# Prayforhanluo/HiCHap_master

Measured on AMD Instinct MI355X. Metric: ICE iterations/sec on 10 kb whole-genome matrix (also nnz*iters/sec), higher is better.
Workload: dtype f64; 1 GPU; hg19-10kb-diploid-wholegenome; n_bins=607282, nnz_upper=4998527599, resolution_bp=10000, parallelism=single GPU, entries_stored=9997055198, slots_u32=160483740, slots_u16=3332512024, payload_bytes=14837255808, tiles=88993, units=88985, hbm_bytes_matrix=15785038153

## Files before the change

### hichap_master_amd/csrc/ice.hip

```cpp
#include <algorithm>
#include <chrono>
#include <functional>
#include <cmath>
#include <limits>

#include "ice_internal.hpp"

namespace hh {
constexpr int kThreads = 256;

constexpr int kSweepThreads = 512;
constexpr int kSweepWaves = kSweepThreads / 64;
constexpr int kFlatU = 8;
static_assert(kFlatU == kFlatIlvU, "k_sweep_flatw walks the interleaved layout's runs");

__device__ __forceinline__ double lds_b(const double* bl, uint32_t byteoff) {
    return *reinterpret_cast<const double*>(reinterpret_cast<const char*>(bl) + byteoff);
}

__device__ __forceinline__ void tile_dot(const uint4 v, const double* __restrict__ bl, double& a0, double& a1) {
    const uint32_t w[4] = {v.x, v.y, v.z, v.w};
    double x[4];
#pragma unroll
    for (int i = 0; i < 4; ++i) x[i] = lds_b(bl, w[i] & 0xFFFFu);
// ... 1179 lines not shown
                {
                    double w[G / 2];
#pragma unroll
                    for (int k = 0; k < G / 2; ++k) w[k] = b0[G / 2 + k];
#pragma unroll
                    for (int j = 0; j < RJ; ++j) acc[j] = band_dot_half<BITS, 1>(sh[j], w, acc[j]);
                }
            }
        }
#pragma unroll
        for (int j = 0; j < RJ; ++j) {
            const double t = wave_sum(acc[j]);
            if (lane == 0 && a[j]) out[r0 + gb + wave + NW * (j0 + j)] = t;
        }
    }
}

template <int ROWS>
struct BandLds {
    static constexpr int L8 = BandGeo<8, ROWS>::LDS, L4 = BandGeo<4, ROWS>::LDS;
    double bl[L8 > L4 ? L8 : L4];
    uint8_t ract[ROWS];
};

template <int ABL, int ROWS, bool DPP = true>
__device__ __forceinline__ void band_any(const BandSegs& S, int rblk, int y, BandLds<ROWS>& L, long long nloc,
                                         long long row_lo, long long n_bins, const uint8_t* __restrict__ act,
                                         const uint16_t* __restrict__ row_group, const double* __restrict__ b,
                                         double* __restrict__ bpart) {
    const int c = S.ord[y];
    int k = 0;
    while (k + 1 < S.n && c >= S.s[k + 1].ch) ++k;
    const BandSeg P = S.s[k];
    if (P.bits == 8)
        band_block<8, ABL, ROWS, DPP>(P, rblk, c - P.ch, L.bl, L.ract, nloc, row_lo, n_bins, act, row_group, b, bpart);
    else
        band_block<4, ABL, ROWS, DPP>(P, rblk, c - P.ch, L.bl, L.ract, nloc, row_lo, n_bins, act, row_group, b, bpart);
}

template <int ABL, int ROWS, bool DPP = true>
__global__ __launch_bounds__(kBandThreads, 4) void k_sweep_bands(BandSegs S, long long nloc, long long row_lo,
                                                              long long n_bins, const uint8_t* __restrict__ act,
                                                              const uint16_t* __restrict__ row_group,
                                                              const double* __restrict__ b,
                                                              double* __restrict__ bpart) {
    __shared__ BandLds<ROWS> L;
    band_any<ABL, ROWS, DPP>(S, blockIdx.x, blockIdx.y, L, nloc, row_lo, n_bins, act, row_group, b, bpart);
}

constexpr int kUbRows = 128;
constexpr int kUbWaves = 4;
constexpr int kUbThreads = 64 * kUbWaves;
constexpr int kUbGroupRows = kUbRows * kUbWaves;
constexpr int kUbChunk = 1008;
constexpr int kUbCols = kUbGroupRows + kUbChunk;
static_assert(kR % kUbGroupRows == 0, "upper-band workgroups must not straddle a shard's row-block boundary");
constexpr int kUbTails = (kUbChunk + kUbGroupRows - 1) / kUbGroupRows;
constexpr int kUbArrs = 2 + kUbTails;
constexpr int kMaxUbChunks = 40;

struct UbSeg {
    const uint8_t* loc;
    const uint8_t* halo;
    long long stride;
    long long dlo;
    int bytes;
    int nc, ch, bits;
};
struct UbSegs {
    UbSeg s[2];
    int n;
    uint8_t ord[kMaxUbChunks];
};
struct UbArgs {
    long long row_lo, row_hi, halo_lo, nloc, g_lo;
    const uint8_t* act;
    const uint16_t* row_group;
    const double* b;
    double* upart;
};

template <int BITS>
struct UbT;
template <>
struct UbT<8> {
    typedef uint4 V;
    static constexpr int LB = 16;
    static __device__ __forceinline__ V zero() { return make_uint4(0u, 0u, 0u, 0u); }
    static __device__ __forceinline__ V ld(const uint8_t* p) { return ld16(reinterpret_cast<const uint4*>(p)); }
    template <int M>
    static __device__ __forceinline__ V shift(const V prev, const V own) {
        if (M == 0) return own;
        constexpr int B = 128 - 8 * M;
        return band_shift_q<B / 32>(prev, own, B % 32);
    }
    static __device__ __forceinline__ uint32_t cnt(const V v, int k) {
        const uint32_t x = k < 4 ? v.x : k < 8 ? v.y : k < 12 ? v.z : v.w;
        return (x >> (8 * (k & 3))) & 0xFFu;
    }
};
typedef uint32_t u32x2 __attribute__((ext_vector_type(2)));
template <>
struct UbT<4> {
    typedef uint2 V;
    static constexpr int LB = 8;
    static __device__ __forceinline__ V zero() { return make_uint2(0u, 0u); }
    static __device__ __forceinline__ V ld(const uint8_t* p) {
        const u32x2 v = *reinterpret_cast<const u32x2*>(p);
        return make_uint2(v.x, v.y);
    }
    template <int M>
    static __device__ __forceinline__ V shift(const V prev, const V own) {
        if (M == 0) return own;
        constexpr int B = 64 - 4 * M, Q = B / 32, R = B % 32;
        const uint32_t d[4] = {prev.x, prev.y, own.x, own.y};
        if (R == 0) return make_uint2(d[Q], d[Q + 1]);
        return make_uint2(__builtin_amdgcn_alignbit(d[Q + 1], d[Q], R), __builtin_amdgcn_alignbit(d[Q + 2], d[Q + 1], R));
    }
    static __device__ __forceinline__ uint32_t cnt(const V v, int k) {
        return ((k < 8 ? v.x : v.y) >> (4 * (k & 7))) & 0xFu;
    }
};

__device__ __forceinline__ double dpp_shl1_d(double x) {
    const int lo = __builtin_amdgcn_update_dpp(0, __double2loint(x), 0x130, 0xF, 0xF, false);
    const int hi = __builtin_amdgcn_update_dpp(0, __double2hiint(x), 0x130, 0xF, 0xF, false);
    return __hiloint2double(hi, lo);
}

__device__ __forceinline__ double ub_cvt(uint32_t x) {
    double r;
    asm volatile("v_cvt_f64_u32 %0, %1" : "=v"(r) : "v"(x));
    return r;
}

__device__ __forceinline__ double ub_bias(const double* __restrict__ b, long long c, long long n) {
    const bool in = c >= 0 && c < n;
    const double v = b[in ? c : 0];
    return (in && v == v) ? v : 0.0;
}

template <int H, int MASK>
__device__ __forceinline__ void ub_halve(double (&v)[8], int lane) {
    const bool hi = (lane & MASK) != 0;
#pragma unroll
    for (int j = 0; j < H; ++j) {
        const double send = hi ? v[j] : v[j + H];
        const double keep = hi ? v[j + H] : v[j];
        v[j] = keep + __shfl_xor(send, MASK, 64);
    }
}
__device__ __forceinline__ double ub_reduce8(double (&v)[8], int lane) {
    ub_halve<4, 1>(v, lane);
    ub_halve<2, 2>(v, lane);
    ub_halve<1, 4>(v, lane);
    double x = v[0];
    x += __shfl_xor(x, 8, 64);
    x += __shfl_xor(x, 16, 64);
    x += __shfl_xor(x, 32, 64);
    return x;
}
__device__ __forceinline__ int ub_reduce8_row(int lane) { return (lane & 1) * 4 + (lane & 2) + ((lane >> 2) & 1); }

__device__ __forceinline__ int ub_pad(int j) { return j + (j >> 4); }
constexpr int kUbWin = kUbCols + kUbCols / 16 + 1;

template <int BITS>
__device__ __forceinline__ void ub_walk(const UbSeg& P, int kc, int chunk, long long r0, const UbArgs& a,
                                        long long n_bins, double* __restrict__ heads, double (&col)[16],
                                        const double* __restrict__ cwin, const double* __restrict__ rowb) {
    using T = UbT<BITS>;
    using V = typename T::V;
    const int lane = threadIdx.x & 63;
    int cb = (kc * kUbChunk + 16 * (lane - 1)) * BITS / 8;
    const bool outside = cb < 0 || cb >= P.bytes;
    const uint32_t msk = (BITS == 8 && outside) ? 0u : ~0u;
    if (outside) cb = P.bytes - T::LB;
    const long long rhi = a.row_hi < r0 + kUbRows ? a.row_hi : r0 + kUbRows;
    const int nv = (int)(rhi - r0);
    const uint8_t* __restrict__ rows = (r0 >= a.row_lo ? P.loc + (r0 - a.row_lo) * P.stride
                                                       : P.halo + (r0 - a.halo_lo) * P.stride) + cb;
    const long long stride = P.stride;
    auto load_row = [&](int i) -> V { return T::ld(rows + (long long)(i < nv ? i : nv - 1) * stride); };
    const int wo = (int)(r0 % kUbGroupRows);
    double w[16];
#pragma unroll
    for (int k = 0; k < 16; ++k) col[k] = 0.0;
    double* __restrict__ R = a.upart + (size_t)(kUbArrs * chunk) * a.nloc;
    V buf[2][4];
#pragma unroll
    for (int j = 0; j < 4; ++j) buf[0][j] = load_row(j);
// ... 5 lines not shown
            {
                const double* src = cwin + ub_pad(wo + 16 * g + 16 * (lane > 0 ? lane - 1 : 0));
#pragma unroll
                for (int k = 0; k < 16; ++k) w[k] = lane ? src[k] : 0.0;
            }
#pragma unroll
            for (int h = 0; h < 2; ++h) {
                double racc[8];
#pragma unroll
                for (int q = 0; q < 2; ++q) {
                    const int bt = 2 * h + q;
#pragma unroll
                    for (int j = 0; j < 4; ++j) buf[(bt + 1) & 1][j] = load_row(16 * g + 4 * (bt + 1) + j);
#pragma unroll
                    for (int j = 0; j < 4; ++j) {
                        const int m = 4 * bt + j, mm = 4 * q + j;
                        V own = buf[bt & 1][j];
                        if (BITS == 8) {
                            uint4& o = *reinterpret_cast<uint4*>(&own);
                            o.x &= msk;
                            o.y &= msk;
                            o.z &= msk;
                            o.w &= msk;
                        }
                        V prev;
                        if (BITS == 8) {
                            const uint4 o = *reinterpret_cast<const uint4*>(&own);
                            const uint4 pv = dpp_shr1(o);
                            prev = *reinterpret_cast<const V*>(&pv);
                        } else {
                            const uint2 o = *reinterpret_cast<const uint2*>(&own);
                            const uint2 pv = make_uint2(__builtin_amdgcn_update_dpp(0u, o.x, 0x138, 0xF, 0xF, false),
                                                        __builtin_amdgcn_update_dpp(0u, o.y, 0x138, 0xF, 0xF, false));
                            prev = *reinterpret_cast<const V*>(&pv);
                        }
                        V sh;
                        switch (m) {
                            case 0: sh = T::template shift<0>(prev, own); break;
                            case 1: sh = T::template shift<1>(prev, own); break;
                            case 2: sh = T::template shift<2>(prev, own); break;
                            case 3: sh = T::template shift<3>(prev, own); break;
                            case 4: sh = T::template shift<4>(prev, own); break;
                            case 5: sh = T::template shift<5>(prev, own); break;
                            case 6: sh = T::template shift<6>(prev, own); break;
                            case 7: sh = T::template shift<7>(prev, own); break;
                            case 8: sh = T::template shift<8>(prev, own); break;
                            case 9: sh = T::template shift<9>(prev, own); break;
                            case 10: sh = T::template shift<10>(prev, own); break;
                            case 11: sh = T::template shift<11>(prev, own); break;
                            case 12: sh = T::template shift<12>(prev, own); break;
                            case 13: sh = T::template shift<13>(prev, own); break;
                            case 14: sh = T::template shift<14>(prev, own); break;
                            default: sh = T::template shift<15>(prev, own); break;
                        }
                        const double br = rowb[wo + 16 * g + m];
                        double a0 = 0.0, a1 = 0.0;
#pragma unroll
                        for (int k = 0; k < 16; k += 2) {
                            const double c0 = ub_cvt(T::cnt(sh, k)), c1 = ub_cvt(T::cnt(sh, k + 1));
                            a0 = fma(c0, w[k], a0);
                            a1 = fma(c1, w[k + 1], a1);
                            col[k] = fma(c0, br, col[k]);
                            col[k + 1] = fma(c1, br, col[k + 1]);
                            asm volatile("" : "+v"(col[k]), "+v"(col[k + 1]), "+v"(a0), "+v"(a1));
                        }
                        racc[mm] = a0 + a1;
                    }
                    __builtin_amdgcn_sched_barrier(0);
                }
                const double s = ub_reduce8(racc, lane);
                const long long r = gb + 8 * h + ub_reduce8_row(lane);
                if (lane < 8 && r < rhi && r >= a.row_lo) R[r - a.row_lo] = s;
            }
        }
        if (lane == 1) {
#pragma unroll
            for (int k = 0; k < 16; ++k) heads[16 * g + k] = col[k];
        }
#pragma unroll
        for (int k = 0; k < 16; ++k) col[k] = dpp_shl1_d(col[k]);
    }
}

__device__ __forceinline__ void ub_group(const UbSegs& S, long long grp, int chunk, const UbArgs& a, long long n_bins,
                                         double* __restrict__ cbuf, double* __restrict__ cwin,
                                         double* __restrict__ rowb) {
    int si = 0;
    while (si + 1 < S.n && chunk >= S.s[si + 1].ch) ++si;
    const UbSeg& P = S.s[si];
    const int kc = chunk - P.ch;
    const long long R0 = grp * kUbGroupRows;
    const int wave = __builtin_amdgcn_readfirstlane(threadIdx.x >> 6), lane = threadIdx.x & 63;
    const long long base = P.dlo + (long long)kc * kUbChunk;
    for (int j = threadIdx.x; j < kUbCols - kUbGroupRows; j += kUbThreads) cbuf[kUbGroupRows + j] = 0.0;
    for (int j = threadIdx.x; j < kUbCols; j += kUbThreads) cwin[ub_pad(j)] = ub_bias(a.b, R0 + base + j, n_bins);
    for (int j = threadIdx.x; j < kUbGroupRows; j += kUbThreads) rowb[j] = ub_bias(a.b, R0 + j, n_bins);
    __syncthreads();
    const long long r0 = R0 + (long long)kUbRows * wave;
    const bool rows_here = r0 < a.row_hi && r0 + kUbRows > a.row_lo;
    const bool cols_here = r0 + base < a.row_hi && r0 + kUbRows + base + kUbChunk > a.row_lo;
    const bool stored = r0 + kUbRows > a.halo_lo && r0 < a.row_hi;
    double col[16];
    double* heads = cbuf + (size_t)kUbRows * wave;
    if ((rows_here || cols_here) && stored) {
        if (P.bits == 8)
            ub_walk<8>(P, kc, chunk, r0, a, n_bins, heads, col, cwin, rowb);
        else
            ub_walk<4>(P, kc, chunk, r0, a, n_bins, heads, col, cwin, rowb);
    } else {
        for (int j = lane; j < kUbRows; j += 64) heads[j] = 0.0;
#pragma unroll
        for (int k = 0; k < 16; ++k) col[k] = 0.0;
    }
    for (int w = 0; w < kUbWaves; ++w) {
        __syncthreads();
        if (wave == w && lane > 0) {
            double* t = cbuf + (size_t)kUbRows * (wave + 1) + 16 * (lane - 1);
#pragma unroll
            for (int k = 0; k < 16; ++k) t[k] += col[k];
        }
    }
    __syncthreads();
    double* __restrict__ base_p = a.upart + (size_t)(kUbArrs * chunk + 1) * a.nloc;
    for (int j = threadIdx.x; j < kUbCols; j += kUbThreads) {
        const long long c = R0 + base + j;
        if (c >= a.row_lo && c < a.row_hi) base_p[(size_t)(j / kUbGroupRows) * a.nloc + (c - a.row_lo)] = cbuf[j];
    }
}

__global__ __launch_bounds__(kUbThreads, 3) void k_sweep_ubands(UbSegs S, UbArgs a, long long n_bins, int xcd) {
    __shared__ double cbuf[kUbCols];
    __shared__ double cwin[kUbWin];
    __shared__ double rowb[kUbGroupRows];
    long long grp = blockIdx.x;
    int y = blockIdx.y;
    if (xcd) {
        const long long nb = (long long)gridDim.x * gridDim.y, b = blockIdx.x + (long long)blockIdx.y * gridDim.x;
        const long long L = xcd_remap(b, nb);
        y = (int)(L % gridDim.y);
        grp = L / gridDim.y;
    }
    ub_group(S, a.g_lo + grp, S.ord[y], a, n_bins, cbuf, cwin, rowb);
}

__global__ void k_ub_halo(const uint8_t* __restrict__ band, const uint8_t* __restrict__ band4, long long W8,
                          long long W4, long long row_lo, long long row_hi, long long halo_lo,
                          uint8_t* __restrict__ h8, uint8_t* __restrict__ h4) {
    const long long nh = row_lo - halo_lo;
    const long long st8 = band_stride(W8), st4 = band4_stride(W8, W4), sg = band4_seg(W8, W4);
    const long long per = W8 + (W4 > W8 ? sg : 0);
    const long long i = (long long)blockIdx.x * blockDim.x + threadIdx.x;
    if (i >= nh * per) return;
    const long long hr = i / per, j = i % per, c = halo_lo + hr;
    if (j < W8) {
        const long long d = j + 1, r = c + d;
        if (r >= row_lo && r < row_hi) h8[hr * st8 + W8 + d] = band[(r - row_lo) * st8 + (W8 - d)];
    } else {
        const long long jb = j - W8;
        uint32_t v = 0;
#pragma unroll
        for (int q = 0; q < 2; ++q) {
            const long long d = W8 + 1 + 2 * jb + q, r = c + d;
            if (d <= W4 && r >= row_lo && r < row_hi) {
                const long long nib = band4_nibble(-d, W8, W4);
                v |= ((band4[(r - row_lo) * st4 + (nib >> 1)] >> (4 * (nib & 1))) & 0xFu) << (4 * q);
            }
        }
        h4[hr * st4 + sg + jb] = (uint8_t)v;
    }
}

static_assert(kBandThreads == kSweepThreads, "one block shape");
template <int NB, int U, int ABL, bool UP>
__global__ __launch_bounds__(kSweepThreads, 4) void k_sweep_all(TileDev T, const uint8_t* __restrict__ act,
                                                              int n_tiled, int n_band, BandSegs S, int band_rb,
                                                              long long nloc, long long row_lo,
                                                              const uint16_t* __restrict__ row_group,
                                                              const double* __restrict__ b, long long n_bins,
                                                              double* __restrict__ part,
                                                              double* __restrict__ bpart,
                                                              unsigned long long* __restrict__ trace) {
    __shared__ __attribute__((aligned(16))) union Lds {
        TiledLds<UP> t;
        FlatLds<UP> f;
        BandLds<64> band;
    } L;
    const int x = blockIdx.x;
    const unsigned long long t0 = trace ? wall_clock64() : 0ull;
    if (x < n_tiled) {
        sweep_tiled_unit<NB, ABL, UP>(T, act, T.u_order[x], b, n_bins, part, L.t);
    } else if (x < n_tiled + n_band) {
        const int y = x - n_tiled;
        band_any<ABL, 64>(S, y % band_rb, y / band_rb, L.band, nloc, row_lo, n_bins, act, row_group, b, bpart);
    } else {
        sweep_flat_unit<U, ABL, UP>(T, act, T.u_order[x - n_band], b, n_bins, part, L.f);
    }
    if (trace) {
        __syncthreads();
        if (threadIdx.x == 0) {
            trace[3 * (size_t)x] = t0;
            trace[3 * (size_t)x + 1] = wall_clock64();
            trace[3 * (size_t)x + 2] = (unsigned long long)__smid();
        }
    }
}

struct UbMarg {
    const double* part;
    int n;
    long long base[kMaxUbChunks];
};
constexpr int kMargThreads = kR;
constexpr int kMargU = 256;

struct TileArgs {
    const int32_t* tile_lo;
    const int32_t* tile_hi;
    const int32_t* tile_group;
    const int32_t* group_tile_ptr;
    const int32_t* blk_tile_ptr;
    double* tile_cnt;
    double* tile_sum;
    double* tile_sq;
    double* g_cnt;
    double* g_sum;
// ... 410 lines not shown
constexpr int kFuseMaxTiles = 128;
}

struct hh_ice {
    hh_matrix* m = nullptr;
    hh_ice_opts o{};
    int64_t n = 0, nloc = 0;
    int32_t G = 1;
    std::vector<int64_t> glo, ghi;
    int32_t n_tiles = 0;
    DBuf<int32_t> tile_lo, tile_hi, tile_group, group_tile_ptr, blk_tile_ptr;
    DBuf<double> bias, marg, part, tile_cnt, tile_sum, tile_sq, g_cnt, g_sum;
    DBuf<unsigned> counter;
    bool stats_fresh = false;
    DBuf<double> bpart;
    int32_t nch = 0;
    int32_t nchu = 0;
    DBuf<double> upart;
    DBuf<uint8_t> halo8, halo4;
    int64_t halo_lo = 0, ub_glo = 0, ub_ghi = 0;
    DBuf<uint8_t> active;
    DBuf<double> g_var, g_mean;
    DBuf<int32_t> g_iters;
    DBuf<uint8_t> g_empty;
    DBuf<long long> rank_rows;
    std::vector<int64_t> h_rank_rows;
    DBuf<unsigned long long> colpart, colacc, bmax, bfix;
    DBuf<double> fix;
    double rmax = 1.0;
    bool rmax_global = false;
    int32_t cx_world = 1, cx_rank = 0;
    int64_t cx_maxlen = 0;
    std::vector<int64_t> cx_rr;
    DBuf<long long> cx_rr_dev;
    hh_reduce_fn cx_fn = nullptr;
    void* cx_user = nullptr;
    hh_allgather_fn cx_ag = nullptr;
    void* cx_ag_user = nullptr;
    DBuf<unsigned long long> cx_send, cx_recv, cx_all;
    int32_t iters_done = 0;
    PinnedBuf<uint8_t> h_active;
    std::vector<hipEvent_t> ev;
    double sweep_ms = 0.0, iter_ms = 0.0;
    int32_t sweep_launches = 0;
    hipStream_t side = nullptr, side2 = nullptr;
    hipEvent_t fork = nullptr, join = nullptr, join2 = nullptr;
    ~hh_ice() {
        for (auto e : ev) (void)hipEventDestroy(e);
        if (join2) (void)hipEventDestroy(join2);
        if (side2) (void)hipStreamDestroy(side2);
        if (fork) (void)hipEventDestroy(fork);
        if (join) (void)hipEventDestroy(join);
        if (side) (void)hipStreamDestroy(side);
    }
    bool full() const { return m->row_lo == 0 && m->row_hi == m->n_bins; }
    TileArgs ta() {
        return TileArgs{tile_lo.p, tile_hi.p, tile_group.p, group_tile_ptr.p, blk_tile_ptr.p, tile_cnt.p,
                        tile_sum.p, tile_sq.p, g_cnt.p, g_sum.p, counter.p};
    }
    bool small_stats() const { return hh::g_fuse_stats == 1 || (hh::g_fuse_stats < 0 && n_tiles <= hh::kFuseMaxTiles); }
    uint8_t* act() { return active.p + (iters_done & 1) * G; }
    uint8_t* nxt() { return active.p + (1 - (iters_done & 1)) * G; }
};

namespace hh {

static int g_sweep_nb = 2;
static int g_band_dpp = 0;
static int g_flatw_waves = 11;
static int g_flatw_waves_up = 8;
static int g_flatw_pipe = 2;
static int g_sweep_ablate = 0;
static int g_band_concurrent = 1;
static int g_split_tiles = 1;
static int g_conc_order = 1;
static int64_t g_conc_min_bytes = 8LL << 30;
static int64_t g_conc_ub_min_bytes = 1LL << 30;
static int g_band_rows = 0;
static int g_band_fused = 1;
static int g_band_lpt = 1;
static int g_uband = 1;
static int64_t g_uband_min_bytes = 128LL << 20;
static int g_ub_xcd = 1;
static int g_sweep_single = -1;
static int g_iter_events = 1;
static int64_t g_single_max_bytes = 1LL << 30;
static unsigned long long* g_trace = nullptr;
static int64_t g_trace_cap = 0, g_trace_n = 0;

template <int NB, int ABL, bool UP>
static void launch_sweep_up(const hh_matrix* m, const TileDev& T, const uint8_t* act, const double* b, double* part,
                            hipStream_t s, hipStream_t s_tiled, int which) {
    const int n_tiled = (int)(m->n_units - m->n_units_flat), n_flat = (int)m->n_units_flat;
    auto tiled = [&] {
        if (!n_tiled) return;
        HH_KTIME("k_sweep_tiled", s_tiled);
        hipLaunchKernelGGL((k_sweep_tiled<NB, ABL, UP>), dim3((unsigned)n_tiled), dim3(kSweepThreads), 0, s_tiled,
                           T, act, n_tiled, b, (long long)m->n_bins, part);
    };
    if (which & 1) tiled();
    if (!(which & 2)) return;
    HH_KTIME(n_flat ? "k_sweep_flat" : nullptr, s);
    if (n_flat && m->n_fgroups) {
        HH_REQUIRE(m->flat_perm, "column-grouped flat tiles without the interleaved layout");
        auto kern = g_flatw_pipe == 2   ? k_sweep_flatw<kFlatU, ABL, 2>
                    : g_flatw_pipe == 1 ? k_sweep_flatw<kFlatU, ABL, 1>
                                        : k_sweep_flatw<kFlatU, ABL, 0>;
        int nw = 8;
        if constexpr (UP) {
            nw = g_flatw_waves_up == 11 ? 11 : 8;
            kern = nw == 11 ? k_sweep_flatw<kFlatU, ABL, 2, 11, true> : k_sweep_flatw<kFlatU, ABL, 2, 8, true>;
        } else {
            if (g_flatw_waves == 10) {
                kern = g_flatw_pipe == 2 ? k_sweep_flatw<kFlatU, ABL, 2, 10> : k_sweep_flatw<kFlatU, ABL, 0, 10>;
                nw = 10;
            } else if (g_flatw_waves == 11) {
                kern = g_flatw_pipe == 2 ? k_sweep_flatw<kFlatU, ABL, 2, 11> : k_sweep_flatw<kFlatU, ABL, 0, 11>;
                nw = 11;
            }
        }
        hipLaunchKernelGGL(kern, dim3((unsigned)m->n_fgroups), dim3(64 * nw), 0, s, T, act, b,
                           (long long)m->n_bins, part);
    } else if (n_flat) {
        hipLaunchKernelGGL((k_sweep_flat<kFlatU, ABL, UP>), dim3((unsigned)n_flat), dim3(kSweepThreads), 0, s, T,
                           act, n_flat, n_tiled, b, (long long)m->n_bins, part);
    }
}

template <int NB, int ABL>
static void launch_sweep(const hh_matrix* m, const TileDev& T, const uint8_t* act, const double* b, double* part,
                         hipStream_t s, hipStream_t s_tiled, int which) {
    if constexpr (kUpperBuild) {
        if (T.upper) return launch_sweep_up<NB, ABL, true>(m, T, act, b, part, s, s_tiled, which);
    }
    launch_sweep_up<NB, ABL, false>(m, T, act, b, part, s, s_tiled, which);
}

template <int ABL>
static void launch_sweep_nb(const hh_matrix* m, const TileDev& T, const uint8_t* act, const double* b, double* part,
                            hipStream_t s, hipStream_t st, int which) {
    switch (g_sweep_nb) {
        case 1: launch_sweep<1, ABL>(m, T, act, b, part, s, st, which); break;
        case 2: launch_sweep<2, ABL>(m, T, act, b, part, s, st, which); break;
        case 8: launch_sweep<8, ABL>(m, T, act, b, part, s, st, which); break;
        default: launch_sweep<4, ABL>(m, T, act, b, part, s, st, which); break;
    }
}

static void sweep(const hh_matrix* m, const TileDev& T, const uint8_t* act, const double* b, double* part,
                  hipStream_t s, hipStream_t s_tiled = nullptr, int which = 3) {
    if (m->n_units == 0) return;
    if (!s_tiled) s_tiled = s;
    switch (g_sweep_ablate) {
        case 1: launch_sweep_nb<1>(m, T, act, b, part, s, s_tiled, which); break;
        case 2: launch_sweep_nb<2>(m, T, act, b, part, s, s_tiled, which); break;
        case 3: launch_sweep_nb<3>(m, T, act, b, part, s, s_tiled, which); break;
        default: launch_sweep_nb<0>(m, T, act, b, part, s, s_tiled, which); break;
    }
    HIP_CHECK(hipGetLastError());
}

static TileDev tdev(const hh_ice* S) { return S->m->dev(S->colpart.p, S->fix.p, S->bfix.p); }

static void band_order(BandSegs& segs, int ch) {
    std::vector<std::pair<long long, int>> w;
    for (int k = 0; k < segs.n; ++k)
        for (int c = 0; c < segs.s[k].nc; ++c) {
            const long long bytes = std::min<long long>(kBandChunkB, segs.s[k].bytes - (long long)c * kBandChunkB);
            w.push_back({g_band_lpt ? -bytes * (8 / segs.s[k].bits) : 0, segs.s[k].ch + c});
        }
    std::stable_sort(w.begin(), w.end(), [](const auto& a, const auto& b) { return a.first < b.first; });
    for (int y = 0; y < ch; ++y) segs.ord[y] = (uint8_t)w[y].second;
}

static int band_segs(const hh_matrix* m, BandSegs& segs) {
    const long long W8 = m->band_w, W4 = m->band_w4;
    segs = BandSegs{};
    int ch = 0;
    auto add = [&](const uint8_t* seg, long long stride, long long bytes, long long dlo, int bits) {
        const int nc = (int)((bytes + kBandChunkB - 1) / kBandChunkB);
        segs.s[segs.n++] = BandSeg{seg, stride, dlo, (int)bytes, nc, ch, bits};
        ch += nc;
    };
    if (W8 > 0) add(m->band.p, band_stride(W8), band_stride(W8), -W8, 8);
    if (W4 > W8) {
        const long long st = band4_stride(W8, W4), sg = band4_seg(W8, W4);
        add(m->band4.p, st, sg, -W4, 4);
        add(m->band4.p + sg, st, sg, W8 + 1, 4);
    }
    HH_REQUIRE(ch <= kMaxBandChunks, "too many band chunks");
    band_order(segs, ch);
    return ch;
}

static int ub_segs(const hh_ice* S, UbSegs& u) {
    const hh_matrix* m = S->m;
    const long long W8 = m->band_w, W4 = m->band_w4;
    u = UbSegs{};
    int ch = 0;
    auto add = [&](const uint8_t* loc, const uint8_t* halo, long long stride, long long dlo, long long bytes,
                   long long slots, int bits) {
        const int nc = (int)((slots + 15 + kUbChunk - 1) / kUbChunk);
        u.s[u.n++] = UbSeg{loc, halo, stride, dlo, (int)bytes, nc, ch, bits};
        ch += nc;
    };
    if (W8 > 0)
        add(m->band.p + W8, S->halo8.p ? S->halo8.p + W8 : nullptr, band_stride(W8), 0, W8 + 16, W8 + 1, 8);
    if (W4 > W8) {
        const long long sg = band4_seg(W8, W4);
        add(m->band4.p + sg, S->halo4.p ? S->halo4.p + sg : nullptr, band4_stride(W8, W4), W8 + 1, sg, W4 - W8, 4);
    }
    HH_REQUIRE(ch <= kMaxUbChunks, "too many upper-band chunks");
    std::vector<std::pair<long long, int>> w;
    for (int k = 0; k < u.n; ++k)
        for (int c = 0; c < u.s[k].nc; ++c) {
            const long long slots = u.s[k].bits == 8 ? W8 + 1 : W4 - W8;
            w.push_back({-std::min<long long>(kUbChunk, slots + 15 - (long long)c * kUbChunk), u.s[k].ch + c});
        }
    std::stable_sort(w.begin(), w.end(), [](const auto& a, const auto& b) { return a.first < b.first; });
    for (int y = 0; y < ch; ++y) u.ord[y] = (uint8_t)w[y].second;
    return ch;
}

static UbArgs ub_args(hh_ice* S) {
    const hh_matrix* m = S->m;
    return UbArgs{m->row_lo, m->row_hi, S->halo_lo, S->nloc, S->ub_glo, S->act(), m->row_group.p, S->bias.p,
                  S->upart.p};
}

static UbMarg ub_marg(const hh_ice* S) {
    UbMarg u{};
    u.part = S->upart.p;
    u.n = S->nchu;
    if (!S->nchu) return u;
    UbSegs segs;
    ub_segs(S, segs);
    for (int k = 0; k < segs.n; ++k)
        for (int c = 0; c < segs.s[k].nc; ++c) u.base[segs.s[k].ch + c] = segs.s[k].dlo + (long long)c * kUbChunk;
    return u;
}

static void sweep_uband(hh_ice* S, hipStream_t s) {
    UbSegs segs;
    const int ch = ub_segs(S, segs);
    const long long ng = S->ub_ghi - S->ub_glo;
    if (!ch || ng <= 0) return;
    HH_KTIME("k_sweep_ubands", s);
    hipLaunchKernelGGL(k_sweep_ubands, dim3((unsigned)ng, (unsigned)ch), dim3(kUbThreads), 0, s, segs, ub_args(S),
                       (long long)S->m->n_bins, g_ub_xcd);
    HIP_CHECK(hipGetLastError());
}

static void sweep_band(hh_ice* S, hipStream_t s) {
    if (S->nchu) {
        if (S->nloc) sweep_uband(S, s);
        return;
    }
    const hh_matrix* m = S->m;
    if (!S->nch || !S->nloc) return;
    BandSegs segs;
    const int ch = band_segs(m, segs);
    const int rows = g_band_rows ? g_band_rows : (((S->nloc + 255) / 256) * ch < 1024 ? 64 : 256);
    const bool abl = g_sweep_ablate == 1;
    auto launch = [&](const BandSegs& L, int nc) {
        const unsigned rb = (unsigned)((S->nloc + rows - 1) / rows);
        auto kern = rows == 64    ? (abl ? k_sweep_bands<1, 64> : k_sweep_bands<0, 64>)
                    : rows == 128 ? (abl ? k_sweep_bands<1, 128> : k_sweep_bands<0, 128>)
                                  : (abl ? k_sweep_bands<1, 256>
                                         : (g_band_dpp ? k_sweep_bands<0, 256, true> : k_sweep_bands<0, 256, false>));
        hipLaunchKernelGGL(kern, dim3(rb, (unsigned)nc), dim3(kBandThreads), 0, s, L, (long long)S->nloc,
                           (long long)m->row_lo, (long long)m->n_bins, S->act(), m->row_group.p, S->bias.p,
                           S->bpart.p);
        HIP_CHECK(hipGetLastError());
    };
    if (g_band_fused) {
        launch(segs, ch);
    } else {
        for (int k = 0; k < segs.n; ++k) {
            BandSegs one{};
            one.s[0] = segs.s[k];
            one.n = 1;
            for (int y = 0; y < segs.s[k].nc; ++y) one.ord[y] = (uint8_t)(segs.s[k].ch + y);
            launch(one, segs.s[k].nc);
        }
    }
}

static void sweep_single(hh_ice* S, hipStream_t s) {
    const hh_matrix* m = S->m;
    BandSegs segs;
    const int ch = (S->nch && S->nloc && !S->nchu) ? band_segs(m, segs) : (segs = BandSegs{}, 0);
    const int band_rb = (int)((S->nloc + 63) / 64);
    const int n_tiled = (int)(m->n_units - m->n_units_flat), n_flat = (int)m->n_units_flat;
    const long long n_band = ch ? (long long)band_rb * ch : 0;
    const long long grid = n_tiled + n_band + n_flat;
    if (S->nchu && S->nloc) sweep_uband(S, s);
    if (!grid) return;
    HH_REQUIRE(grid < (1LL << 31), "sweep grid too large for one launch");
    unsigned long long* trace = grid <= g_trace_cap ? g_trace : nullptr;
    if (trace) g_trace_n = grid;
    auto kern = g_sweep_ablate == 1   ? k_sweep_all<2, kFlatU, 1, false>
                : g_sweep_ablate == 2 ? k_sweep_all<2, kFlatU, 2, false>
                                      : k_sweep_all<2, kFlatU, 0, false>;
    if constexpr (kUpperBuild) {
        if (m->upper && S->colpart.p)
            kern = g_sweep_ablate == 1   ? k_sweep_all<2, kFlatU, 1, true>
                   : g_sweep_ablate == 2 ? k_sweep_all<2, kFlatU, 2, true>
                                         : k_sweep_all<2, kFlatU, 0, true>;
    }
    hipLaunchKernelGGL(kern, dim3((unsigned)grid), dim3(kSweepThreads), 0, s, tdev(S), S->act(), n_tiled,
                       (int)n_band, segs, band_rb, (long long)S->nloc, (long long)m->row_lo, m->row_group.p,
                       S->bias.p, (long long)m->n_bins, S->part.p, S->bpart.p, trace);
    HIP_CHECK(hipGetLastError());
}

static void ensure_side_streams(hh_ice* S) {
    if (S->side) return;
    int cur = 0;
    HIP_CHECK(hipGetDevice(&cur));
    if (cur != S->m->device) HIP_CHECK(hipSetDevice(S->m->device));
    HIP_CHECK(hipStreamCreateWithFlags(&S->side, hipStreamNonBlocking));
    HIP_CHECK(hipEventCreateWithFlags(&S->fork, hipEventDisableTiming));
    HIP_CHECK(hipEventCreateWithFlags(&S->join, hipEventDisableTiming));
    HIP_CHECK(hipStreamCreateWithFlags(&S->side2, hipStreamNonBlocking));
    HIP_CHECK(hipEventCreateWithFlags(&S->join2, hipEventDisableTiming));
    if (cur != S->m->device) HIP_CHECK(hipSetDevice(cur));
}

static void marg_weighted(hh_ice* S, double* out, hipStream_t s, bool timed, int slot) {
    hh_matrix* m = S->m;
    const bool up = m->upper && S->colpart.p;
    const bool shard_x = up && S->cx_world > 1;
// ... 144 lines not shown
    const std::vector<double> all = gather ? gather(marg) : marg;
    std::vector<double> logm;
    for (double x : all)
        if (x > 0) logm.push_back(std::log(x));
    const double med = np_median(logm);
    std::vector<double> dev(logm.size());
    for (size_t k = 0; k < logm.size(); ++k) dev[k] = std::fabs(logm[k] - med);
    const double cutoff = std::exp(med - S->o.mad_max * np_median(dev));
    for (int64_t i = 0; i < S->n; ++i)
        if (marg[i] < cutoff) bias[i] = 0.0;
    upload_pinned_sync(S->bias.p, bias.data(), (size_t)S->n, s);
}

extern "C" {

int hh_tune(const char* key, int64_t value) {
    return guard([&] {
        HH_REQUIRE(key, "null key");
        const std::string k(key);
        if (k == "sweep_nb") {
            HH_REQUIRE(value == 1 || value == 2 || value == 4 || value == 8, "sweep_nb must be 1, 2, 4 or 8");
            g_sweep_nb = (int)value;
        } else if (k == "sweep_ablate") {
            HH_REQUIRE(value >= 0 && value <= 3, "sweep_ablate must be 0, 1, 2 or 3");
            g_sweep_ablate = (int)value;
        } else if (k == "band4_density_pct" || k == "band8_big_pct") {
            HH_REQUIRE(value >= 1 && value <= 100, "percent in [1, 100]");
            (k == "band4_density_pct" ? g_band4_density : g_band8_big) = (double)value / 100.0;
        } else if (k == "band4") {
            HH_REQUIRE(value == 0 || value == 1, "band4 in {0, 1}");
            g_band4 = value;
        } else if (k == "flat_cols") {
            HH_REQUIRE(value >= -1 && value <= 1, "flat_cols in {-1 (auto), 0, 1}");
            g_flat_cols = value;
        } else if (k == "flatw_pipe") {
            HH_REQUIRE(value >= 0 && value <= 2, "flatw_pipe in {0, 1, 2}");
            g_flatw_pipe = (int)value;
        } else if (k == "band_dpp") {
            HH_REQUIRE(value == 0 || value == 1, "band_dpp in {0, 1}");
            g_band_dpp = (int)value;
        } else if (k == "flatw_u") {
            HH_REQUIRE(value == 8, "flatw_u: 8 (the interleaved flat layout's run length)");
        } else if (k == "flatw_waves_up") {
            HH_REQUIRE(value == 8 || value == 11, "flatw_waves_up in {8, 11}");
            g_flatw_waves_up = (int)value;
        } else if (k == "upper_tiles") {
            HH_REQUIRE(value >= -1 && value <= 1, "upper_tiles in {-1 (auto), 0, 1}");
            HH_REQUIRE(kUpperBuild || value != 1,
                       "upper-triangle tiles need the 4096-column build (libhichap_hip_up.so, -DHH_KWBITS=12)");
            g_upper_tiles = value;
        } else if (k == "flat_max") {
            HH_REQUIRE(value >= 0 && value <= 255, "flat_max in [0, 255]");
            g_flat_max = value;
        } else if (k == "unit_entries") {
            HH_REQUIRE(value == 0 || (value >= 4096 && value <= (1 << 24)), "unit_entries must be 0 (auto) or in [4096, 2^24]");
            g_unit_entries = value;
        } else if (k == "flat_defer") {
            HH_REQUIRE(value == 0 || value == 1, "flat_defer in {0, 1}");
            g_flat_defer = (int)value;
        } else if (k == "unit_lpt") {
            HH_REQUIRE(value >= 0 && value <= 2, "unit_lpt in {0, 1, 2}");
            g_unit_lpt = value;
        } else if (k == "unit_lpt_lists") {
            HH_REQUIRE(value >= 0 && value <= 3, "unit_lpt_lists in [0, 3]");
            g_unit_lpt_lists = value;
        } else if (k == "tile_cost") {
            HH_REQUIRE(value >= 0 && value <= (1 << 20), "tile_cost in [0, 2^20] payload words");
            g_tile_cost = value;
        } else if (k == "parse_ablate") {
            HH_REQUIRE(value >= 0 && value <= 3, "parse_ablate in [0, 3]");
            g_parse_ablate = (int)value;
        } else if (k == "flatw_waves") {
            HH_REQUIRE(value == 8 || value == 10 || value == 11, "flatw_waves: 8, 10 or 11");
            g_flatw_waves = (int)value;
        } else if (k == "flat_group") {
            HH_REQUIRE(value >= 0 && value <= 256, "flat_group: 0 (auto) .. 256");
            g_flat_group = value;
        } else if (k == "uband") {
            HH_REQUIRE(value >= 0 && value <= 2, "uband: 0 (off), 1 (auto) or 2 (always)");
            g_uband = (int)value;
        } else if (k == "ub_xcd") {
            HH_REQUIRE(value == 0 || value == 1, "ub_xcd: 0 or 1");
            g_ub_xcd = (int)value;
        } else if (k == "uband_min_bytes") {
            HH_REQUIRE(value >= 0, "uband_min_bytes >= 0");
            g_uband_min_bytes = value;
        } else if (k == "band_w") {
            HH_REQUIRE(value >= -1 && value <= kBandMaxW && (value <= 0 || value % 16 == 0),
                       "band_w: -1 (auto), 0 (off) or a multiple of 16 <= 16384");
            g_band_w = value;
        } else if (k == "conc_min_bytes") {
            HH_REQUIRE(value >= 0, "conc_min_bytes >= 0");
            g_conc_min_bytes = value;
        } else if (k == "syrk_split") {
            HH_REQUIRE(value >= -1 && value <= 64, "syrk_split in [-1, 64]");
            g_syrk_split = (int)value;
        } else if (k == "band_lpt") {
            HH_REQUIRE(value == 0 || value == 1, "band_lpt in {0, 1}");
            g_band_lpt = (int)value;
        } else if (k == "fuse_stats") {
            HH_REQUIRE(value >= -1 && value <= 2, "fuse_stats in {-1, 0, 1, 2}");
            g_fuse_stats = (int)value;
        } else if (k == "conc_order") {
            HH_REQUIRE(value >= 0 && value <= 2, "conc_order in {0, 1, 2}");
            g_conc_order = (int)value;
        } else if (k == "split_tiles") {
            HH_REQUIRE(value == 0 || value == 1, "split_tiles in {0, 1}");
            g_split_tiles = (int)value;
        } else if (k == "pca_method") {
            HH_REQUIRE(value == 0 || value == 1, "pca_method in {0, 1}");
            g_pca_method = (int)value;
        } else if (k == "host_build") {
            HH_REQUIRE(value == 0 || value == 1, "host_build in {0, 1}");
            g_host_build = value;
        } else if (k == "build_debug") {
            g_build_debug = value;
        } else if (k == "pca_debug") {
            g_pca_debug = (int)value;
        } else if (k == "conc_ub_min_bytes") {
            HH_REQUIRE(value >= 0, "conc_ub_min_bytes >= 0");
            g_conc_ub_min_bytes = value;
        } else if (k == "ortho_lowsync") {
            g_ortho_lowsync = value ? 1 : 0;
        } else if (k == "ortho_grid_cap") {
            HH_REQUIRE(value >= 0 && value <= 64, "ortho_grid_cap in [0, 64]");
            g_ortho_grid_cap = (int)value;
        } else if (k == "symvc_rows") {
            HH_REQUIRE(value >= 16 && value <= 1024 && value % 16 == 0, "symvc_rows in [16, 1024], a multiple of 16");
            g_symvc_rows = (int)value;
        } else if (k == "symvc_out") {
            g_symvc_out = value ? 1 : 0;
        } else if (k == "twostep_budget_mb") {
            HH_REQUIRE(value >= 0, "twostep_budget_mb >= 0 (0: the free device memory)");
            g_twostep_budget = value << 20;
        } else if (k == "twostep_devglue") {
            g_twostep_devglue = value ? 1 : 0;
        } else if (k == "symvc_stream") {
            g_symvc_stream = value ? 1 : 0;
        } else if (k == "ortho_abort_test") {
            HH_REQUIRE(value >= 0 && value <= 2, "ortho_abort_test in {0, 1, 2}");
            g_ortho_abort_test = (int)value;
        } else if (k == "pca_coop") {
            HH_REQUIRE(value == 0 || value == 1, "pca_coop in {0, 1}");
            g_pca_coop = (int)value;
        } else if (k == "cor_sym") {
            HH_REQUIRE(value >= 0 && value <= 3, "cor_sym in {0, 1, 2, 3}");
            g_cor_sym = (int)value;
        } else if (k == "ortho_tpb") {
            HH_REQUIRE(value == 0 || value == 1 || value == 2 || value == 4 || value == 8,
                       "ortho_tpb in {0 (auto), 1, 2, 4, 8}");
            g_ortho_tpb = (int)value;
        } else if (k == "ortho_min_tpb") {
            HH_REQUIRE(value == 1 || value == 2, "ortho_min_tpb in {1, 2}");
            g_ortho_min_tpb = (int)value;
        } else if (k == "pca_p") {
            HH_REQUIRE(value >= 2 && value <= 8, "pca_p in [2, 8]");
            g_pca_p = (int)value;
        } else if (k == "rank_lds_buckets") {
            HH_REQUIRE(value >= 0 && value <= 8192, "rank_lds_buckets in [0, 8192]");
            g_rank_lds_buckets = (int)value;
        } else if (k == "band_rows") {
            HH_REQUIRE(value == 0 || value == 64 || value == 128 || value == 256,
                       "band_rows in {0 (auto), 64, 128, 256}");
            g_band_rows = (int)value;
        } else if (k == "sweep_trace") {
            HH_REQUIRE(value >= 0 && value < (1LL << 31), "sweep_trace: block capacity >= 0");
// ... 600 lines not shown
```

Before: 331.9 ICE iterations/s.

## Add buffer-load double-buffered band walk with LDS transpose reduction

Adds a second walker for the uniform-band sweep kernel, selected by default through a new ub_walk knob. It loads rows with raw buffer loads, using a clamped descriptor so out-of-range lanes need no branches, and double-buffers row loads across batches. Out-of-band lanes read padded zero entries in LDS instead of taking branches. Row sums are reduced through a per-wave LDS transpose plus swizzle and bpermute, replacing the old DPP reduction. The intent is to hide load latency and cut per-row reduction cost, at the price of extra LDS, which may reduce occupancy, and more register pressure.

Result: no change. 333.7 ICE iterations/s (median of 6 runs) (+0.5%).

```diff
diff --git a/hichap_master_amd/csrc/ice.hip b/hichap_master_amd/csrc/ice.hip
--- a/hichap_master_amd/csrc/ice.hip
+++ b/hichap_master_amd/csrc/ice.hip
@@ -1285,12 +1285,17 @@
 
 template <int BITS>
 struct UbT;
+typedef uint32_t u32x2 __attribute__((ext_vector_type(2)));
 template <>
 struct UbT<8> {
     typedef uint4 V;
     static constexpr int LB = 16;
     static __device__ __forceinline__ V zero() { return make_uint4(0u, 0u, 0u, 0u); }
     static __device__ __forceinline__ V ld(const uint8_t* p) { return ld16(reinterpret_cast<const uint4*>(p)); }
+    static __device__ __forceinline__ V ldb(__amdgpu_buffer_rsrc_t rs, uint32_t vo, uint32_t so) {
+        const u32x4 v = __builtin_amdgcn_raw_buffer_load_b128(rs, (int)vo, (int)so, 0);
+        return make_uint4(v.x, v.y, v.z, v.w);
+    }
     template <int M>
     static __device__ __forceinline__ V shift(const V prev, const V own) {
         if (M == 0) return own;
@@ -1302,7 +1307,6 @@
         return (x >> (8 * (k & 3))) & 0xFFu;
     }
 };
-typedef uint32_t u32x2 __attribute__((ext_vector_type(2)));
 template <>
 struct UbT<4> {
     typedef uint2 V;
@@ -1310,6 +1314,10 @@
     static __device__ __forceinline__ V zero() { return make_uint2(0u, 0u); }
     static __device__ __forceinline__ V ld(const uint8_t* p) {
         const u32x2 v = *reinterpret_cast<const u32x2*>(p);
+        return make_uint2(v.x, v.y);
+    }
+    static __device__ __forceinline__ V ldb(__amdgpu_buffer_rsrc_t rs, uint32_t vo, uint32_t so) {
+        const u32x2 v = __builtin_amdgcn_raw_buffer_load_b64(rs, (int)vo, (int)so, 0);
         return make_uint2(v.x, v.y);
     }
     template <int M>
@@ -1481,9 +1489,156 @@
     }
 }
 
+constexpr int kUbZero = 16;
+constexpr int kUbRedRow = 64 + 1;
+constexpr int kUbRed = 8 * kUbRedRow;
+
+__device__ __forceinline__ uint32_t ub_shr1(uint32_t x) {
+    return (uint32_t)__builtin_amdgcn_update_dpp(0, (int)x, 0x138, 0xF, 0xF, true);
+}
+__device__ __forceinline__ double ub_shl1_d(double x) {
+    const int lo = __builtin_amdgcn_update_dpp(0, __double2loint(x), 0x130, 0xF, 0xF, true);
+    const int hi = __builtin_amdgcn_update_dpp(0, __double2hiint(x), 0x130, 0xF, 0xF, true);
+    return __hiloint2double(hi, lo);
+}
+template <int PAT>
+__device__ __forceinline__ double ub_swz_d(double x) {
+    const int lo = __builtin_amdgcn_ds_swizzle(__double2loint(x), PAT);
+    const int hi = __builtin_amdgcn_ds_swizzle(__double2hiint(x), PAT);
+    return __hiloint2double(hi, lo);
+}
+__device__ __forceinline__ double ub_bperm_d(int addr, double x) {
+    const int lo = __builtin_amdgcn_ds_bpermute(addr, __double2loint(x));
+    const int hi = __builtin_amdgcn_ds_bpermute(addr, __double2hiint(x));
+    return __hiloint2double(hi, lo);
+}
+
+template <int BITS>
+__device__ __forceinline__ void ub_walk2(const UbSeg& P, int kc, int chunk, long long r0, const UbArgs& a,
+                                         double* __restrict__ heads, double (&col)[16],
+                                         const double* __restrict__ cwin, const double* __restrict__ rowb,
+                                         double* __restrict__ red) {
+    using T = UbT<BITS>;
+    using V = typename T::V;
+    constexpr int NW = T::LB / 4, PER = 32 / BITS;
+    const int lane = threadIdx.x & 63;
+    int cb = (kc * kUbChunk + 16 * (lane - 1)) * BITS / 8;
+    const bool outside = cb < 0 || cb >= P.bytes;
+    if (outside) cb = P.bytes - T::LB;
+    const uint32_t co = (uint32_t)cb;
+    const long long rhi = a.row_hi < r0 + kUbRows ? a.row_hi : r0 + kUbRows;
+    const int nv = (int)(rhi - r0);
+    const uint8_t* rp = r0 >= a.row_lo ? P.loc + (r0 - a.row_lo) * P.stride : P.halo + (r0 - a.halo_lo) * P.stride;
+    const uint32_t stride = (uint32_t)P.stride;
+    const __amdgpu_buffer_rsrc_t rs = __builtin_amdgcn_make_buffer_rsrc(
+        const_cast<uint8_t*>(rp), 0, (int)((uint32_t)(nv - 1) * stride + (uint32_t)P.bytes), 0x00020000);
+    uint32_t ro = 0;
+    int left = nv - 1;
+    auto next_row = [&]() -> V {
+        const V v = T::ldb(rs, co, ro);
+        ro += left > 0 ? stride : 0u;
+        --left;
+        return v;
+    };
+    const int wo = (int)(r0 % kUbGroupRows);
+    const bool zw = lane == 0 || (BITS == 8 && outside);
+    const bool zr = BITS == 8 && outside;
+    const double* wsrc = cwin + (zw ? kUbWin : ub_pad(wo + 16 * (lane - 1)));
+    const double* rsrc = rowb + (zr ? kUbGroupRows : wo);
+    const int wstep = zw ? 0 : 17, rstep = zr ? 0 : 16;
+    double* const rput = red + lane;
+    const double* const rget = red + (lane & 7) * kUbRedRow + (lane & ~7);
+    const int a32 = (lane ^ 32) << 2;
+    double w[16];
+#pragma unroll
+    for (int k = 0; k < 16; ++k) col[k] = 0.0;
+    double* __restrict__ Rl = a.upart + (size_t)(kUbArrs * chunk) * a.nloc + (r0 - a.row_lo + lane);
+    const int slim = (r0 >= a.row_lo && lane < 8) ? lane : (1 << 30);
+    constexpr int NB = BITS == 8 ? 4 : 8;
+    V buf[2][NB];
+#pragma unroll
+    for (int j = 0; j < NB; ++j) buf[0][j] = next_row();
+    const int ng = (nv + 15) / 16;
+#pragma unroll 1
+    for (int g = 0; g < kUbRows / 16; ++g) {
+        if (g < ng) {
+#pragma unroll
+            for (int k = 0; k < 16; ++k) w[k] = wsrc[k];
+            double racc[8];
+#pragma unroll
+            for (int bt = 0; bt < 16 / NB; ++bt) {
+                {
+#pragma unroll
+                    for (int j = 0; j < NB; ++j) buf[(bt + 1) & 1][j] = next_row();
+#pragma unroll
+                    for (int j = 0; j < NB; ++j) {
+                        const int m = NB * bt + j, mm = m & 7;
+                        const V own = buf[bt & 1][j];
+                        uint32_t d[2 * NW];
+                        if (BITS == 8) {
+                            const uint4 o = *reinterpret_cast<const uint4*>(&own);
+                            const uint32_t ow[4] = {o.x, o.y, o.z, o.w};
+#pragma unroll
+                            for (int i = 0; i < NW; ++i) d[i] = ub_shr1(ow[i % 4]), d[NW + i] = ow[i % 4];
+                        } else {
+                            const uint2 o = *reinterpret_cast<const uint2*>(&own);
+                            const uint32_t ow[2] = {o.x, o.y};
+#pragma unroll
+                            for (int i = 0; i < NW; ++i) d[i] = ub_shr1(ow[i % 2]), d[NW + i] = ow[i % 2];
+                        }
+                        auto cnt = [&](int k) -> uint32_t {
+                            const int e = 16 - m + k;
+                            return (d[e / PER] >> (BITS * (e % PER))) & ((1u << BITS) - 1u);
+                        };
+                        const double br = rsrc[m];
+                        double a0 = 0.0, a1 = 0.0;
+#pragma unroll
+                        for (int k = 0; k < 16; k += 2) {
+                            const double c0 = ub_cvt(cnt(k)), c1 = ub_cvt(cnt(k + 1));
+                            a0 = fma(c0, w[k], a0);
+                            a1 = fma(c1, w[k + 1], a1);
+                            col[k] = fma(c0, br, col[k]);
+                            col[k + 1] = fma(c1, br, col[k + 1]);
+                            asm volatile("" : "+v"(col[k]), "+v"(col[k + 1]), "+v"(a0), "+v"(a1));
+                        }
+                        racc[mm] = a0 + a1;
+                    }
+                    __builtin_amdgcn_sched_barrier(0);
+                }
+                if ((NB * (bt + 1)) % 8 != 0) continue;
+                const int h = (NB * (bt + 1)) / 8 - 1;
+#pragma unroll
+                for (int i = 0; i < 8; ++i) rput[i * kUbRedRow] = racc[i];
+                __builtin_amdgcn_fence(__ATOMIC_RELEASE, "wavefront");
+                __builtin_amdgcn_wave_barrier();
+                __builtin_amdgcn_fence(__ATOMIC_ACQUIRE, "wavefront");
+                double x[8];
+#pragma unroll
+                for (int i = 0; i < 8; ++i) x[i] = rget[i];
+                __builtin_amdgcn_fence(__ATOMIC_RELEASE, "wavefront");
+                __builtin_amdgcn_wave_barrier();
+                double s = ((x[0] + x[1]) + (x[2] + x[3])) + ((x[4] + x[5]) + (x[6] + x[7]));
+                s += ub_swz_d<0x201F>(s);
+                s += ub_swz_d<0x401F>(s);
+                s += ub_bperm_d(a32, s);
+                if (slim < nv - 16 * g - 8 * h) Rl[16 * g + 8 * h] = s;
+            }
+        }
+        wsrc += wstep;
+        rsrc += rstep;
+        if (lane == 1) {
+#pragma unroll
+            for (int k = 0; k < 16; ++k) heads[16 * g + k] = col[k];
+        }
+#pragma unroll
+        for (int k = 0; k < 16; ++k) col[k] = ub_shl1_d(col[k]);
+    }
+}
+
+template <int WALK>
 __device__ __forceinline__ void ub_group(const UbSegs& S, long long grp, int chunk, const UbArgs& a, long long n_bins,
                                          double* __restrict__ cbuf, double* __restrict__ cwin,
-                                         double* __restrict__ rowb) {
+                                         double* __restrict__ rowb, double* __restrict__ red) {
     int si = 0;
     while (si + 1 < S.n && chunk >= S.s[si + 1].ch) ++si;
     const UbSeg& P = S.s[si];
@@ -1494,6 +1649,7 @@
     for (int j = threadIdx.x; j < kUbCols - kUbGroupRows; j += kUbThreads) cbuf[kUbGroupRows + j] = 0.0;
     for (int j = threadIdx.x; j < kUbCols; j += kUbThreads) cwin[ub_pad(j)] = ub_bias(a.b, R0 + base + j, n_bins);
     for (int j = threadIdx.x; j < kUbGroupRows; j += kUbThreads) rowb[j] = ub_bias(a.b, R0 + j, n_bins);
+    if (WALK && threadIdx.x < kUbZero) cwin[kUbWin + threadIdx.x] = rowb[kUbGroupRows + threadIdx.x] = 0.0;
     __syncthreads();
     const long long r0 = R0 + (long long)kUbRows * wave;
     const bool rows_here = r0 < a.row_hi && r0 + kUbRows > a.row_lo;
@@ -1502,10 +1658,17 @@
     double col[16];
     double* heads = cbuf + (size_t)kUbRows * wave;
     if ((rows_here || cols_here) && stored) {
-        if (P.bits == 8)
+        if (WALK) {
+            double* wred = red + (size_t)kUbRed * wave;
+            if (P.bits == 8)
+                ub_walk2<8>(P, kc, chunk, r0, a, heads, col, cwin, rowb, wred);
+            else
+                ub_walk2<4>(P, kc, chunk, r0, a, heads, col, cwin, rowb, wred);
+        } else if (P.bits == 8) {
             ub_walk<8>(P, kc, chunk, r0, a, n_bins, heads, col, cwin, rowb);
-        else
+        } else {
             ub_walk<4>(P, kc, chunk, r0, a, n_bins, heads, col, cwin, rowb);
+        }
     } else {
         for (int j = lane; j < kUbRows; j += 64) heads[j] = 0.0;
 #pragma unroll
@@ -1527,10 +1690,12 @@
     }
 }
 
+template <int WALK>
 __global__ __launch_bounds__(kUbThreads, 3) void k_sweep_ubands(UbSegs S, UbArgs a, long long n_bins, int xcd) {
     __shared__ double cbuf[kUbCols];
-    __shared__ double cwin[kUbWin];
-    __shared__ double rowb[kUbGroupRows];
+    __shared__ __attribute__((aligned(16))) double cwin[kUbWin + (WALK ? kUbZero : 0)];
+    __shared__ __attribute__((aligned(16))) double rowb[kUbGroupRows + (WALK ? kUbZero : 0)];
+    __shared__ __attribute__((aligned(16))) double red[WALK ? kUbRed * kUbWaves : 1];
     long long grp = blockIdx.x;
     int y = blockIdx.y;
     if (xcd) {
@@ -1539,7 +1704,7 @@
         y = (int)(L % gridDim.y);
         grp = L / gridDim.y;
     }
-    ub_group(S, a.g_lo + grp, S.ord[y], a, n_bins, cbuf, cwin, rowb);
+    ub_group<WALK>(S, a.g_lo + grp, S.ord[y], a, n_bins, cbuf, cwin, rowb, red);
 }
 
 __global__ void k_ub_halo(const uint8_t* __restrict__ band, const uint8_t* __restrict__ band4, long long W8,
@@ -2116,6 +2281,7 @@
 static int g_uband = 1;
 static int64_t g_uband_min_bytes = 128LL << 20;
 static int g_ub_xcd = 1;
+static int g_ub_walk = 1;
 static int g_sweep_single = -1;
 static int g_iter_events = 1;
 static int64_t g_single_max_bytes = 1LL << 30;
@@ -2280,8 +2446,8 @@
     const long long ng = S->ub_ghi - S->ub_glo;
     if (!ch || ng <= 0) return;
     HH_KTIME("k_sweep_ubands", s);
-    hipLaunchKernelGGL(k_sweep_ubands, dim3((unsigned)ng, (unsigned)ch), dim3(kUbThreads), 0, s, segs, ub_args(S),
-                       (long long)S->m->n_bins, g_ub_xcd);
+    hipLaunchKernelGGL(g_ub_walk ? k_sweep_ubands<1> : k_sweep_ubands<0>, dim3((unsigned)ng, (unsigned)ch),
+                       dim3(kUbThreads), 0, s, segs, ub_args(S), (long long)S->m->n_bins, g_ub_xcd);
     HIP_CHECK(hipGetLastError());
 }
 
@@ -2592,6 +2758,9 @@
         } else if (k == "ub_xcd") {
             HH_REQUIRE(value == 0 || value == 1, "ub_xcd: 0 or 1");
             g_ub_xcd = (int)value;
+        } else if (k == "ub_walk") {
+            HH_REQUIRE(value == 0 || value == 1, "ub_walk: 0 or 1");
+            g_ub_walk = (int)value;
         } else if (k == "uband_min_bytes") {
             HH_REQUIRE(value >= 0, "uband_min_bytes >= 0");
             g_uband_min_bytes = value;
```
